# labgem/pangenomeNEM

Hardware: AMD Instinct MI355X
Metric: em_family_x_organism_cells_per_sec (higher is better)
Workload: dtype f32 chains with f64 intermediates (reference arithmetic); int32 popcounts in the M-step; 1 GPU; BASELINE configs[1]: 20000 families x 500 organisms, K=3, beta=0.5, contiguity graph (path + 5% chords, weights 1..8), ncem/sk_/pk; U-shaped family-frequency spectrum (Beta(0.3, 0.3) per family), default .m init; families_total=20000, families_per_gpu=20000, organisms=500, K=3, parallelism=1 GPU

## Files before the change

### include/nem_mi355x.h

```cpp
#ifndef NEM_MI355X_H
#define NEM_MI355X_H

#include <stdint.h>

#ifdef __cplusplus
extern "C" {
#endif

int nem(const char* Fname,
        const int nk,
        const char* algo,
        const float beta,
        const char* convergence,
        const float convergence_th,
        const char* format,
        const int it_max,
        const int dolog,
        const char* model_family,
        const char* proportion,
        const char* dispersion,
        const int init_mode);

typedef struct nemgpu_engine nemgpu_engine;

// ... 276 lines not shown
int nemgpu_ff_table(double l1, double l0, uint32_t* q0_256, uint32_t* q1_256);

float nemgpu_chain_host(const double* x, long long n, float init, int mode);
float nemgpu_repeat_add_host(float x, long long times, int mode);
int nemgpu_chain_device(const double* x, long long n, float init, int device, float* out);
float nemgpu_halfsum_host(const float* x, int n, int mode, int* stepped);
int nemgpu_halfsum_device(const float* x, int n, int waves, int device, float* out);
int nemgpu_halfsum_profile(const float* x, int n, int waves, int device, double us[5]);
int nemgpu_map_margin_host(const double* cinum, int n, int K, int* out);
int nemgpu_map_margin_device(const double* pkf, const float* ctx, int n, int K, float beta, int use_nei, int device, int* out);

void nemgpu_release_cached(void);

int nemgpu_set_graph_policy(nemgpu_engine* e, int capture_on_first);
int nemgpu_graph_counters(const nemgpu_engine* e, int out[4]);
int nemgpu_random_start_counters(const nemgpu_engine* e, int out[4]);

int nemgpu_set_stream(nemgpu_engine* e, void* hip_stream);

typedef struct nemgpu_gff nemgpu_gff;
int nemgpu_gff_info(int* tile_bytes, int* n_thresholds, int* thresholds);
int nemgpu_gff_create(nemgpu_gff** out, int device, const char* families_text, long long bytes, int hash_bits, int* n_families);
int nemgpu_gff_family_spans(const nemgpu_gff* h, int32_t* spans);
int nemgpu_gff_batch(nemgpu_gff* h, const char* text, long long bytes, const int32_t* file_start, const int32_t* file_end, int n_files,
                     int infer_singletons, int* n_genes, int* n_contigs, unsigned long long* error);
int nemgpu_gff_fetch(const nemgpu_gff* h, int32_t* file, int32_t* start, int32_t* end, int32_t* span_off, int32_t* span_len, int32_t* fam,
                     int32_t* contig, int32_t* fasta_off);
int nemgpu_gff_number(nemgpu_gff* h, const int32_t* name, const int32_t* org, int g, int n_names, int n_orgs, int lim_occurence, int32_t* genes,
                      int32_t* order, uint8_t* repeated, int* n_used);
int nemgpu_gff_stage_ms(const nemgpu_gff* h, float* ms);
// ... 7 lines not shown
```

### pangenomenem_amd/csrc/nem_engine.hip

```cpp
#include <hip/hip_runtime.h>
#include <dlfcn.h>
#include <pthread.h>
#include <unistd.h>

#include <algorithm>
#include <climits>
#include <atomic>
#include <cfloat>
#include <chrono>
#include <cmath>
#include <cstdio>
#include <cstdlib>
#include <cstring>
#include <condition_variable>
#include <deque>
#include <functional>
#include <map>
#include <string>
#include <mutex>
#include <thread>
#include <vector>

#include "nem_internal.hpp"
#include "nem_ff.hpp"
// ... 127 lines not shown
    double *crit2_lfi = nullptr, *crit2_lzi = nullptr;
    char* crit_pair_dev = nullptr;

    uint32_t sweep_counter = 0;
    int iters = 0, converged = 0, emptyk = 0, status = NEMGPU_OK;
    int zero_density = 0, first_zero = -1, sweep_rounds = 0;
    bool masks_valid = false;
    bool flags_clean = false;

    GraphCache batch_graphs{2 * 3 * 8 * 8, true, true};
    bool use_graphs = true;
    bool shadow_verify = true;
    int flag_sets = 1, fset = 0;
    bool round_counts = true;
    bool start_fused = true;
    int* stats_slot[2] = {};
    int* stats_last = nullptr;
    float* par_copy[3] = {}; double* pkfki_copy[3] = {}; float* logpkfki_copy[3] = {};
    int round_batch = 3;
    int rounds_iter = 2;
    int deep_iters = 2;
    uint8_t fz_need[kFzPositions] = {}; uint8_t fz_init_need = 0;
    int run_deep_used = 0; bool run_tracked = false;
    bool capture_first = false;
    int n_plain = 0, n_captured = 0, n_replayed = 0, n_host_rounds = 0;
    int ff_mode = -1;
    bool fused_update() const
    {
        return d <= kFusedMaxD && (cfg.disper == NEMGPU_DISP_KD || cfg.disper == NEMGPU_DISP_K_);
    }
// ... 441 lines not shown
    e->flags_clean = true;
    e->density_fresh = true;
    return NEMGPU_OK;
}

struct SweepCtx {
    SweepArgs a{};
    bool use_nei = false;
    bool multi = false;
    int r = 0;
    int checked = 0;
    int slot_base = 0;
    bool post = false; bool post_moved = false; CtrlArgs post_ctrl{};
    SweepArgs* hold = nullptr;
    int* count_into = nullptr;
};

int clear_sweep_flags(nemgpu_engine* e)
{
    if (current_recorder()) launch_fill(e->iter_flags() + FLAG_MOVED, kSweepFlagWords, 0, e->stream);
    else HIPCHK(hipMemsetAsync(e->iter_flags() + FLAG_MOVED, 0, kSweepFlagWords * sizeof(int), e->stream));
    e->flags_clean = true;
    return NEMGPU_OK;
}

int ensure_draw_window(nemgpu_engine* e, long lo, long count)
{
    if (e->draw_valid && e->draw_tab0 <= lo && lo + count <= e->draw_tab0 + e->draw_cap) return NEMGPU_OK;
    if (e->draw_borrowed) {
        e->draw_borrowed = false; e->draw_valid = false; e->draw_tab = nullptr; e->draw_cap = 0;
// ... 62 lines not shown
    const int r0 = c.r;
    for (int b = 0; b < count; b++, c.r++) {
        const int r = c.r;
        const int gb = (r == 0) ? P : ((r - 1) % 2 == 0 ? Q : R);
        const int ob = (r % 2 == 0) ? Q : R;
        if (ncem) {
            c.a.lab_old = e->lab[P]; c.a.lab_guess = e->lab[gb]; c.a.lab_out = e->lab[ob];
            c.a.tie_cnt_guess = e->tie_cnt[gb]; c.a.tie_cnt_out = e->tie_cnt[ob];
        } else { c.a.c_old = e->cbuf[P]; c.a.c_guess = e->cbuf[gb]; c.a.c_out = e->cbuf[ob]; }
        c.a.flags = e->round_flags(c.slot_base + r);
        c.a.fold_ticket = e->sweep_next + 32;
        c.a.prev_changed = (r == r0) ? nullptr : (e->round_flags(c.slot_base + r - 1) + FLAG_CHANGED);
        c.a.stop = e->stop_ptr;
        c.a.post_on = 0;
        c.a.post_stats = nullptr;
        if (c.hold != nullptr && c.post && ncem && r0 == 0 && count >= 2 && b >= count - 2) {
            c.a.post_on = 1; c.a.post_skip_guess = (r % 2 == 1) ? 1 : 0;
            c.a.post_nw64 = e->nw64; c.a.post_mask = e->mask; c.a.post_flags = e->iter_flags();
            if (b == count - 2) {
                c.a.post_from_guess = 0; c.a.post_moved = c.post_moved ? 1 : 0; c.a.post_no_masks = 0; c.a.post_ctrl = CtrlArgs{};
                if (c.count_into != nullptr) { c.a.post_stats = c.count_into; c.a.post_xt = e->xt; c.a.post_D = e->d; }
            } else {
                c.a.post_from_guess = 1; c.a.post_moved = 0; c.a.post_no_masks = 1; c.a.post_ctrl = c.post_ctrl;
                *c.hold = c.a;
                continue;
            }
        } else if (c.post && ncem && r0 == 0 && b == count - 1) {
            c.a.post_on = 1; c.a.post_from_guess = (r % 2 == 1) ? 1 : 0; c.a.post_moved = c.post_moved ? 1 : 0;
            c.a.post_skip_guess = c.a.post_from_guess;
            c.a.post_nw64 = e->nw64; c.a.post_mask = e->mask; c.a.post_flags = e->iter_flags(); c.a.post_ctrl = c.post_ctrl;
// ... 16 lines not shown
    a.pkfki = e->pkfki;
    a.tie_rule = e->cfg.tie_rule; a.tie_seed = e->cfg.tie_seed; a.map_full = e->map_margin ? 0 : 1; a.sweep_id = e->sweep_counter++;
    a.sweep_id_ptr = (e->stop_ptr != nullptr && !id_by_value) ? e->sweep_next : nullptr;
    if (e->libc()) {
        if (e->stop_ptr == nullptr) { int r = ensure_draw_window(e, e->draws, draw_need(e)); if (r) return r; }
        sweep_draw_args(e, a, e->stop_ptr == nullptr);
    }
    return NEMGPU_OK;
}

int sweep_enqueue(nemgpu_engine* e, float beta, SweepCtx& c, bool id_by_value = false, const CtrlArgs* post_ctrl = nullptr,
                  bool post_moved = false, int slot_base = 0, int rounds = 0, SweepArgs* hold = nullptr, int* count_into = nullptr)
{
    c = SweepCtx();
    c.slot_base = slot_base;
    if (post_ctrl != nullptr && e->ncem()) {
        c.post = true; c.post_moved = post_moved; c.post_ctrl = *post_ctrl; c.hold = hold;
        c.count_into = hold != nullptr ? count_into : nullptr;
    }
    { int r = sweep_setup(e, beta, c, id_by_value); if (r) return r; }
    if (!e->flags_clean) { int r = clear_sweep_flags(e); if (r) return r; }
    e->flags_clean = false;
    return sweep_launch_rounds(e, c, c.multi ? (rounds > 0 ? rounds : e->round_batch) : 1);
}

int sweep_complete(nemgpu_engine* e, SweepCtx& c, int* rounds_out, bool* extra, bool flags_ready = false, bool grow = false)
{
    int done_at = -1;
    if (extra) *extra = false;
    for (;;) {
// ... 205 lines not shown
{
    const char* v = getenv("NEM_MI355X_LIBC_INIT");
    return !(v && strcmp(v, "host") == 0);
}

static int init_beta_rounds(const nemgpu_engine* e)
{
    int n = std::max<int>(e->round_batch, (!e->ncem() && current_recorder() == nullptr) ? e->fz_init_need : 0);
    if (e->libc()) n = e->libc_rb;
    else if (e->ncem() && current_recorder() == nullptr && e->init_rounds_ncem >= 2) n = e->init_rounds_ncem;
    return n;
}

bool shadow_engine(const nemgpu_engine* e);

int enqueue_init(nemgpu_engine* e, bool defer_ctrl, SweepArgs* hold = nullptr, int* count_into = nullptr)
{
    int r;
    FinishArgs t = finish_args(e, 0, nullptr);
    t.reset_prop = e->prop0; t.reset_center = e->center0; t.reset_disp = e->disp0;
    t.reset_ctrl = e->ctrl(); t.reset_ctrl_words = C_WORDS; t.reset_sweep_next = e->sweep_next;
    if (hold != nullptr && count_into != nullptr) { t.zero_stats = count_into; t.n_zero_stats = e->k + e->k * e->d; }
    e->cur = 0;
    if (e->start_fused && shadow_engine(e)) {
        launch_density_start(t, e->xws, e->n, e->npad, e->pkfki, e->logpkfki, e->iter_flags() + FLAG_MOVED, kSweepFlagWords, e->stream);
        HIPCHK(hipGetLastError());
        e->tables_fresh = false;
        e->flags_clean = true; e->density_fresh = true;
    } else {
        launch_finish(t, e->stream);
        HIPCHK(hipGetLastError());
        e->tables_fresh = true; e->density_fresh = false;
        if ((r = do_density(e))) return r;
    }
    SweepCtx c0, c1;
    e->sweep_counter = 0;
    const bool libc = e->libc();
    const int ra = libc ? e->libc_ra : 1;
    if ((r = sweep_enqueue(e, 0.0f, c0, true, nullptr, false, kRoundCap - ra, libc ? ra : 0))) return r;
    e->flags_clean = true;
    e->cur = 1;
    CtrlArgs ca{};
    ca.ctrl = e->ctrl(); ca.iter_flags = e->iter_flags(); ca.round0 = e->round_flags(0); ca.n_rounds = init_beta_rounds(e);
    ca.param_fix = e->cfg.param_fix; ca.use_nei = ((e->has_graph && e->cfg.beta != 0.0f) || e->libc()) ? 1 : 0; ca.cvtest = e->cfg.cvtest;
    ca.ncem = e->ncem() ? 1 : 0; ca.cvthres = e->cfg.cvthres; ca.sweep_next = e->sweep_next; ca.ticket = e->sweep_next + 32;
    ca.draw_ctl = e->libc() ? e->draw_ctl : nullptr;
    ca.is_init = 1;
    ca.blind = e->round_flags(kRoundCap - ra);
    ca.blind_rounds = libc ? ra : 0;
    const bool defer = defer_ctrl && e->ncem() && !e->cfg.param_fix && hold == nullptr;
    CtrlArgs none{};
    if (libc) e->draw_extra_once = e->round_flags(kRoundCap - 1) + FLAG_NTIES;
    if ((r = sweep_enqueue(e, e->cfg.beta, c1, true, e->ncem() ? (defer ? &none : &ca) : nullptr, false, 0, ca.n_rounds, hold,
                           count_into))) return r;
// ... 488 lines not shown
    return enqueue();
}

int iterate_pipelined(nemgpu_engine* e, int n_iters, bool with_init)
{
    int r;
    LoopCursor lc;
    if ((r = loop_begin(e, lc, n_iters, with_init))) return r;
    if (lc.first && e->libc() && !libc_init_pipelined()) {
        if ((r = libc_init(e))) return r;
        lc.first = false;
    }
    while (loop_wants_batch(e, lc)) {
        if ((r = batch_plan(e, lc))) return r;
        const int cur0 = e->cur; const uint32_t sweep_counter0 = e->sweep_counter;
        Graphed how;
        r = run_graphed(e, lc.g < 8 ? &e->batch_graphs : nullptr, {(uint64_t)lc.batch_first, (uint64_t)lc.base, (uint64_t)lc.g, (uint64_t)lc.deep},
                        2, e->stream, [&]() { return batch_enqueue(e, lc, true); },
                        [&]() { e->cur = cur0; e->sweep_counter = sweep_counter0; }, &how);
        e->n_plain += how == Graphed::plain;
        e->n_captured += how == Graphed::captured;
        e->n_replayed += how == Graphed::replayed || (how == Graphed::captured && r == NEMGPU_OK);
        if (r) return r;
        HIPCHK(hipStreamSynchronize(e->stream));
        if ((r = batch_finish(e, lc))) return r;
    }
    return NEMGPU_OK;
}

int criteria(nemgpu_engine* e, float crit6[6], int buf);

int iterate_crit(nemgpu_engine* e, int n_iters, bool with_init)
{
    int r;
// ... 721 lines not shown
    e->n_total = n_total; e->n_true = n_total; e->d = d; e->k = k; e->lo = site_lo; e->hi = site_hi; e->n = site_hi - site_lo;
    e->device = device;
    e->npad = (e->n + 255) / 256 * 256;
    e->dpad = (d + 63) / 64 * 64;
    e->W = e->dpad / 32;
    e->wf = (d + 31) / 32;
    e->nw64 = (e->n + 63) / 64;
    e->cfg.algo = NEMGPU_ALGO_NCEM; e->cfg.beta = 0.5f; e->cfg.disper = NEMGPU_DISP_K_; e->cfg.propor = NEMGPU_PROP_K;
    e->cfg.cvtest = NEMGPU_CV_CLAS; e->cfg.cvthres = 1e-8f; e->cfg.it_max = 100; e->cfg.param_fix = 0;
    e->cfg.tie_rule = NEMGPU_TIE_HASH; e->cfg.tie_seed = 0;
    if (const char* g = getenv("NEM_MI355X_GRAPHS")) e->use_graphs = (g[0] != '0');
    if (const char* g = getenv("NEM_MI355X_SHADOW_VERIFY")) e->shadow_verify = (g[0] != '0');
    e->flag_sets = e->shadow_verify ? 3 : 1;
    if (const char* g = getenv("NEM_MI355X_ROUND_COUNTS")) e->round_counts = (g[0] != '0');
    if (const char* g = getenv("NEM_MI355X_START_FUSED")) e->start_fused = (g[0] != '0');
    if (const char* g = getenv("NEM_MI355X_ROUNDS")) e->round_batch = std::max(2, std::min(kRoundBatchMax, atoi(g)));
    if (const char* g = getenv("NEM_MI355X_ROUNDS_ITER")) e->rounds_iter = std::max(2, std::min(e->round_batch, atoi(g)));
    e->rounds_iter = std::min(e->rounds_iter, e->round_batch);
    if (const char* g = getenv("NEM_MI355X_FAULT_INJECT")) e->fault_inject = !strcmp(g, "fuzzy_pc") ? 1 : 0;
    if (const char* g = getenv("NEM_MI355X_FF")) e->ff_mode = (g[0] == '0') ? 0 : (g[0] == '1') ? 1 : -1;
    if (const char* g = getenv("NEM_MI355X_FF_BATCH")) e->ff_batch = (g[0] != '0');
    if (const char* g = getenv("NEM_MI355X_MAP_MARGIN")) e->map_margin = (g[0] != '0');
    if (const char* g = getenv("NEM_MI355X_SORT")) e->use_sort = (g[0] != '0');
    if (hip_stream) { e->stream = (hipStream_t)hip_stream; e->own_stream = false; }
    else {
        if (pool_stream_get(device, &e->stream) != hipSuccess) { delete e; set_error("hipStreamCreate failed"); return NEMGPU_E_DEVICE; }
        e->own_stream = true;
    }
    int r = NEMGPU_OK;
    alloc_for(e);
// ... 2791 lines not shown

int nemgpu_set_graph_policy(nemgpu_engine* e, int capture_on_first)
{
    if (!e) return NEMGPU_E_FUNCARG;
    e->capture_first = capture_on_first != 0;
    return NEMGPU_OK;
}

int nemgpu_graph_counters(const nemgpu_engine* e, int out[4])
{
    if (!e || !out) return NEMGPU_E_FUNCARG;
    out[0] = e->n_plain; out[1] = e->n_captured; out[2] = e->n_replayed; out[3] = e->n_host_rounds;
    return NEMGPU_OK;
}

int nemgpu_random_start_counters(const nemgpu_engine* e, int out[4])
{
    if (!e || !out) return NEMGPU_E_FUNCARG;
    out[0] = e->rs_rounds; out[1] = e->rs_lockstep; out[2] = e->rs_alone; out[3] = e->rs_redone;
    return NEMGPU_OK;
}

int nemgpu_set_stream(nemgpu_engine* e, void* hip_stream)
{
    if (!e || !hip_stream) return NEMGPU_E_FUNCARG;
    if (e->own_stream && e->stream) { (void)hipStreamSynchronize(e->stream); (void)hipStreamDestroy(e->stream); }
    e->stream = (hipStream_t)hip_stream;
    e->own_stream = false;
    drop_graphs(e);
    return NEMGPU_OK;
// ... 113 lines not shown
```

### pangenomenem_amd/csrc/nem_kernels.hpp

```cpp
#pragma once
#include <hip/hip_runtime.h>
#include <cstdint>
#include <cstring>
#include <type_traits>
#include <vector>

#include "../../include/nem_mi355x.h"

namespace nemk {

constexpr int kMaxKernelK = 32;
constexpr int kTicketWords = 32 * 33;
constexpr double kEpsilonD = 1e-20;

enum { FLAG_CHANGED = 0, FLAG_NZERO = 1, FLAG_FIRSTZERO = 2, FLAG_NTIES = 3, FLAG_ROUND_STRIDE = 4 };
enum { FLAG_EMPTYK = 0, FLAG_EMPTY_PROP = 1, FLAG_FAULT = 2, FLAG_MOVED = 3, FLAG_ITER_STRIDE = 4 };

enum { C_STOP = 0, C_FOLD = 1, C_ITERS = 10, C_COMMITS = 2, C_STATUS = 3, C_EMPTYK = 4, C_CONVERGED = 5, C_NEED_ROUNDS = 6,
       C_SWEEP_ROUNDS = 7, C_NZERO = 8, C_FIRSTZERO = 9, C_DRAWS = 11, C_DEEP = 12, C_DRAWS_INIT = 13, C_INIT_ROUNDS = 14, C_WORDS = 16 };

struct CtrlArgs {
    int* ctrl; const int* iter_flags; const int* round0;
    int n_rounds;
    int param_fix, use_nei, cvtest, ncem; float cvthres;
// ... 5 lines not shown
    const int* blind;
    int blind_rounds;
    int* draw_ctl;
    const uint8_t* q_tot;
};
void launch_ctrl(const CtrlArgs& a, hipStream_t s);

struct SweepArgs {
    int n_local, lo, n_total, K, npad, use_nei;
    const int* nei_ptr; const int* nei_idx; const float* nei_w;
    float beta;
    const double* pkfki;
    const uint8_t* lab_old; const uint8_t* lab_guess; uint8_t* lab_out;
    const float* c_old; const float* c_guess; float* c_out;
    int tie_rule; uint32_t tie_seed; uint32_t sweep_id;
    const int* sweep_id_ptr;
    int* flags;
    const int* prev_changed;
    const int* stop;
    const uint8_t* flags_in; int n_ranks, slot_stride, slot_pad;
    int post_on, post_from_guess, post_moved, post_nw64, post_skip_guess;
    int post_no_masks;
    uint64_t* post_mask; int* post_flags;
    CtrlArgs post_ctrl;
    uint8_t* publish_byte; int* publish_ticket;
    int* fold_ticket;
    const uint32_t* draw_tab; int draw_tab_len, draw_base, draw_tab0;
    const int* draw_ctl; const int* draw_extra;
    const int* tie_cnt_guess; int* tie_cnt_out;
    const uint8_t* rank_tot_in; int rank_index; uint8_t* rank_tot_out;
    int spb;
    int* post_stats; const uint64_t* post_xt; int post_D;
    int map_full;
};
struct LabelsPostArgs { int n_local, lo, K, nw64; const uint8_t* lab_new; const uint8_t* lab_old; uint64_t* mask; int* flags;
                        const int* stop; CtrlArgs ca; };
struct CountsArgs { int K, D, nw64; const uint64_t* xt; const uint64_t* mask; int* stats; const int* stop; CtrlArgs prev_ctrl; };
struct FuzzyArgs { int n, npad, K, D; const uint32_t* xw; const uint64_t* xt; int nw64; const float* c; float* nbobs_k;
                   float* in0; float* in1; float* inh_k; int* lastz; int* any1; float* center; float* iner; const int* stop;
                   float* ct; int ctpad;
                   float* chk;
                   int* fault;
                   int inject; };
struct ConvFuzzyArgs { size_t m; const float* c; const float* cold; float thres; int* flags; const int* stop; CtrlArgs ca; };
struct OnehotArgs { int n, K; const uint8_t* lab; float* c; };
struct CritArgs { int n, K, npad; const int* nei_ptr; const int* nei_idx; const float* nei_w; int use_nei; float beta;
// ... 121 lines not shown
```

### pangenomenem_amd/csrc/nem_sweep.hip

```cpp
#include <hip/hip_runtime.h>
#include <algorithm>
#include <cstdio>
#include <cstdlib>

#include "nem_kernels.hpp"
#include "nem_sweep_dev.hpp"

namespace nemk {

template <int KT, bool NCEM, int BS, bool LIBC = false, bool COUNT = false>
__global__ __launch_bounds__(BS) void k_sweep(SweepArgs a) { sweep_body<KT, NCEM, BS, LIBC, COUNT>(a, blockIdx.x, gridDim.x); }
template <int KT, bool NCEM, int BS, bool LIBC = false>
__global__ __launch_bounds__(BS) void k_sweep_b(const void* arr, int stride, const int* gx) { NEM_B_HEAD(SweepArgs) sweep_body<KT, NCEM, BS, LIBC>(a, blockIdx.x, nblk); }

static int sweep_variant(int K, bool ncem, bool big, bool libc) { return (K >= 1 && K <= 10 ? K : 0) | (ncem ? 16 : 0) | (big ? 32 : 0) | (libc && ncem ? 64 : 0); }

template <bool BATCHED>
static void sweep_dispatch(int variant, dim3 grid, unsigned bdim, hipStream_t s, const SweepArgs* a, const void* arr, int stride, const int* gx)
{
    const int kt = variant & 15; const bool ncem = (variant & 16) != 0, big = (variant & 32) != 0, libc = (variant & 64) != 0;
    dim3 block(bdim);
    auto launch = [&](auto KT, auto NC, auto BS, auto LC) {
        if (BATCHED) hipLaunchKernelGGL((k_sweep_b<decltype(KT)::value, decltype(NC)::value, decltype(BS)::value, decltype(LC)::value>), grid, block, 0, s, arr, stride, gx);
        else hipLaunchKernelGGL((k_sweep<decltype(KT)::value, decltype(NC)::value, decltype(BS)::value, decltype(LC)::value>), grid, block, 0, s, *a);
    };
    auto modes = [&](auto KT, auto BS) {
// ... 15 lines not shown
        const int per_block = (n_local + 256 * waves_of_blocks - 1) / (256 * waves_of_blocks);
        bs = std::min(1024, std::max(256, (per_block + 63) / 64 * 64));
    }
    if (big_out) *big_out = big;
    return bs;
}

void launch_sweep(const SweepArgs& a0, bool ncem, hipStream_t s)
{
    bool big = false;
    SweepArgs a = a0;
    const int bs = sweep_block_sites(a.n_local, a.K, &big);
    a.spb = big ? bs : 0;
    dim3 grid((a.n_local + bs - 1) / bs);
    const int variant = sweep_variant(a.K, ncem, big, a.tie_rule == NEMGPU_TIE_LIBC);
    if (a.post_stats != nullptr) {
        if (!(current_recorder() == nullptr && ncem && !big && a.K >= 1 && a.K <= 10 && a.tie_rule != NEMGPU_TIE_LIBC &&
              a.post_on && !a.post_no_masks && a.post_D >= 1 && a.post_D <= kFusedMaxD)) {
            fprintf(stderr, "launch_sweep: no counting round for this shape\n");
            abort();
        }
        dispatch_k<1, 10>(a.K, [&](auto KT) {
            hipLaunchKernelGGL((k_sweep<decltype(KT)::value, true, 256, false, true>), grid, dim3(256), 0, s, a);
        });
        return;
    }
    if (record_op(OP_SWEEP, variant, grid, (unsigned)bs, a)) return;
    sweep_dispatch<false>(variant, grid, (unsigned)bs, s, &a, nullptr, 0, nullptr);
}

// ... 49 lines not shown
```

### pangenomenem_amd/csrc/nem_sweep_dev.hpp

```cpp
#pragma once
#include <hip/hip_runtime.h>
#include <cstdint>

#include "nem_kernels.hpp"
#include "nem_map.hpp"

namespace nemk {

#ifdef NEM_PHASE_PROF
static __device__ unsigned long long g_sweep_phase[16];
#define NEM_SWEEP_PHASE(i) do { if (bx == 0 && threadIdx.x == 0) g_sweep_phase[(COUNT ? 8 : 0) + (i)] = wall_clock64(); } while (0)
#define NEM_SWEEP_PHASE_TAKE(t) const unsigned long long t = wall_clock64()
#define NEM_SWEEP_PHASE_PUT(i, t) do { if (bx == 0 && threadIdx.x == 0) g_sweep_phase[(COUNT ? 8 : 0) + (i)] = t; } while (0)
#else
#define NEM_SWEEP_PHASE(i) do { } while (0)
#define NEM_SWEEP_PHASE_TAKE(t) do { } while (0)
#define NEM_SWEEP_PHASE_PUT(i, t) do { } while (0)
#endif

__host__ __device__ inline uint32_t mix32(uint32_t seed, uint32_t sweep, uint32_t site)
{
    uint32_t h = seed * 0x9E3779B1u + sweep * 0x85EBCA77u + site * 0xC2B2AE3Du + 0x27D4EB2Fu;
    h ^= h >> 16; h *= 0x7FEB352Du;
    h ^= h >> 15; h *= 0x846CA68Bu;
// ... 243 lines not shown
constexpr int kLabMask = 0x7F, kLabDrew = 0x80;
constexpr int kTabShort = 1 << 30;
constexpr int kInnerCap = 64;

__device__ __forceinline__ int wave_sum_i32(int v)
{
    v += __builtin_amdgcn_update_dpp(0, v, 0xB1, 0xF, 0xF, false);
    v += __builtin_amdgcn_update_dpp(0, v, 0x4E, 0xF, 0xF, false);
    v += __builtin_amdgcn_update_dpp(0, v, 0x141, 0xF, 0xF, false);
    v += __builtin_amdgcn_update_dpp(0, v, 0x140, 0xF, 0xF, false);
    v += __builtin_amdgcn_update_dpp(0, v, 0x142, 0xA, 0xF, false);
    v += __builtin_amdgcn_update_dpp(0, v, 0x143, 0xC, 0xF, false);
    return __builtin_amdgcn_readlane(v, 63);
}

template <int KT, bool NCEM, int BS, bool LIBC = false, bool COUNT = false>
__device__ __forceinline__ void sweep_body(const SweepArgs& a, const int bx, const int nblk)
{
    static_assert(!COUNT || (NCEM && BS == 256 && !LIBC && KT > 0), "the counting round: NCEM, 256 sites per block");
    static_assert(C_STOP == 0 && C_FOLD == 1, "one 8-byte load");
    NEM_SWEEP_PHASE_TAKE(t_entry);
    const int spb = (BS > 256 && a.spb > 0) ? a.spb : BS;
    const int i = bx * spb + threadIdx.x;
    const bool active = (int)threadIdx.x < spb && i < a.n_local;
    const int gi = a.lo + (active ? i : 0);
    const int K = KT > 0 ? KT : a.K;
    constexpr int KA = KT > 0 ? KT : kMaxKernelK;
    int my_guess = 0, my_old = 0, my_new = 255;
    int blk_cnt_guess = 0;
    constexpr int kCntRows = COUNT ? kFusedMaxD / BS : 1;
    uint64_t xs[kCntRows][4];
    double pkf[NCEM ? KA : 1];
    int nb = 0, ne = 0;
    int fold_hint = 0;
// ... 4 lines not shown
            const int w0 = 4 * bx;
#pragma unroll
            for (int q = 0; q < kCntRows; q++) {
                const int d = (int)threadIdx.x + q * BS;
#pragma unroll
                for (int w = 0; w < 4; w++)
                    xs[q][w] = (d < a.post_D && w0 + w < a.post_nw64) ? a.post_xt[(size_t)d * a.post_nw64 + w0 + w] : 0ull;
            }
        }
#pragma unroll
        for (int k = 0; k < KA; k++) if (k < K) pkf[k] = active ? a.pkfki[(size_t)k * a.npad + i] : 0.0;
        if (active && a.use_nei) { nb = a.nei_ptr[i]; ne = a.nei_ptr[i + 1]; }
        const int* some = reinterpret_cast<const int*>(a.pkfki);
        int2 sf = *reinterpret_cast<const int2*>(a.stop != nullptr ? a.stop : some);
        int pc = *(a.prev_changed != nullptr ? a.prev_changed : some);
        if (active) { my_guess = a.lab_guess[gi]; my_old = a.lab_old[gi] & kLabMask; }
        if (a.stop == nullptr) sf = make_int2(0, 0);
        if (a.prev_changed == nullptr) pc = 1;
        __atomic_signal_fence(__ATOMIC_SEQ_CST);
        asm volatile("" :: "s"(pc));
        if (sf.x) return;
        fold_hint = sf.y;
        skip = (pc == 0);
    } else {
        if (a.stop != nullptr) {
            const int2 sf = *reinterpret_cast<const int2*>(a.stop);
            if (sf.x) return;
            fold_hint = sf.y;
        }
        skip = (a.prev_changed != nullptr && *a.prev_changed == 0);
    }
// ... 7 lines not shown
    if (skip && !(NCEM && a.post_on)) {
        if (a.publish_byte != nullptr && bx == 0 && threadIdx.x == 0) *a.publish_byte = 0;
        if (LIBC && a.prev_changed != nullptr && bx == 0 && threadIdx.x == 0) a.flags[FLAG_NTIES] = a.prev_changed[FLAG_NTIES - FLAG_CHANGED];
        return;
    }
    __shared__ int s_nzero, s_first;
    __shared__ int s_chg, s_mov;
    constexpr int kExpTab = 64;
    __shared__ double s_exp[NCEM ? kExpTab : 1];
    __shared__ __attribute__((aligned(16))) uint8_t s_lab[NCEM ? BS : 1];
    __shared__ uint64_t s_drew[BS / 64];
    bool zero_density = false;
    bool changed = false;
    __shared__ int s_anydrew;
    if (threadIdx.x == 0) { s_nzero = 0; s_first = 0; s_chg = 0; s_mov = 0; s_anydrew = 0; }
    if (NCEM) s_lab[threadIdx.x] = (uint8_t)my_guess;
    if (NCEM && a.use_nei && !skip && threadIdx.x < kExpTab) s_exp[threadIdx.x] = exp((double)a.beta * (double)(float)threadIdx.x);
    __shared__ int s_lower;
    if (LIBC && !skip && threadIdx.x < 64 && a.tie_cnt_guess != nullptr) {
        int part = 0;
        for (int b = threadIdx.x; b < bx; b += 64) part += a.tie_cnt_guess[b];
        part = wave_sum_i32(part);
        if (threadIdx.x == 0) {
            if (a.rank_tot_in != nullptr)
                for (int r = 0; r < a.rank_index; r++) part += *reinterpret_cast<const int*>(a.rank_tot_in + (size_t)r * a.slot_stride);
            s_lower = part;
        }
    }
    bool blk_drew = false;
    if (LIBC) blk_drew = __syncthreads_or((my_guess & kLabDrew) != 0) != 0;
// ... 3 lines not shown
    if (NCEM) {
    constexpr bool libc = LIBC;
    constexpr bool kMapShort = KT >= 1 && KT <= 7;
    const int blk_lo = a.lo + bx * spb;
    int dyn[4]; float wn[4]; int fl[4];
#pragma unroll
    for (int u = 0; u < 4; u++) { dyn[u] = -1; wn[u] = 0.0f; fl[u] = 255; }
    if (active && !skip && a.use_nei) {
        int jn[4];
#pragma unroll
        for (int u = 0; u < 4; u++) {
            const bool ok = nb + u < ne;
            jn[u] = ok ? a.nei_idx[nb + u] : gi;
            wn[u] = ok ? a.nei_w[nb + u] : 0.0f;
        }
#pragma unroll
        for (int u = 0; u < 4; u++) {
            if (nb + u < ne) {
                if (jn[u] < gi && jn[u] >= blk_lo) dyn[u] = jn[u] - blk_lo;
                else fl[u] = ((jn[u] < gi) ? a.lab_guess[jn[u]] : a.lab_old[jn[u]]) & kLabMask;
            }
        }
    }
    const bool long_row = ne - nb > 4;
    NEM_SWEEP_PHASE(3);
    int lower_draws = -1;
    bool tab_short = false;
    int cur = my_guess;
    int seen[4] = {-1, -1, -1, -1};
    uint64_t seen_drew = ~0ull; int seen_wave_draws = -1;
    for (int it = 0; it < kInnerCap; it++) {
        int below_in_block = 0;
        uint64_t drew_lt = 0;
        if (libc && blk_drew) {
            const uint64_t bal = __ballot((s_lab[threadIdx.x] & kLabDrew) != 0);
            if ((threadIdx.x & 63) == 0) s_drew[threadIdx.x >> 6] = bal;
// ... 17 lines not shown
                for (int k = 0; k < KA; k++) ctx[k] = 0.0f;
#pragma unroll
                for (int u = 0; u < 4; u++) {
                    seen[u] = lab[u];
                    if (nb + u < ne) {
#pragma unroll
                        for (int k = 0; k < KA; k++)
                            if (k < K) ctx[k] = ctx[k] + ((lab[u] == k) ? wn[u] : -0.0f);
                    }
                }
                for (int t = nb + 4; t < ne; t++) {
                    const int j = a.nei_idx[t];
                    const float wt = a.nei_w[t];
                    int l;
                    if (j < gi && j >= blk_lo) l = s_lab[j - blk_lo] & kLabMask;
                    else l = ((j < gi) ? a.lab_guess[j] : a.lab_old[j]) & kLabMask;
#pragma unroll
                    for (int k = 0; k < KA; k++)
                        if (k < K) ctx[k] = ctx[k] + ((l == k) ? wt : -0.0f);
                }
                float cf[KA];
                int kmax = 0;
                bool clear = false;
                if constexpr (kMapShort) {
                    double cinum[KA];
                    const double cum = local_cinum<KA>(a, K, pkf, ctx, cinum, s_exp, kExpTab);
                    zero_density = !(cum > 0);
                    clear = !a.map_full && map_clear_row<KA>(cinum, K, cum, kmax);
                    if (!clear) map_normalise<KA>(cinum, K, cum, cf);
                } else zero_density = local_proba<KA>(a, K, pkf, ctx, cf, s_exp, kExpTab);
// ... 99 lines not shown
    int post_lab = 255;
    if (NCEM && a.post_on) {
        int moved = 0;
        if (active) {
            if (skip) post_lab = (a.post_skip_guess ? my_guess : (int)a.lab_out[gi]) & kLabMask;
            else post_lab = a.post_from_guess ? (my_guess & kLabMask) : (my_new != 255 ? my_new : ((int)a.lab_out[gi] & kLabMask));
            if (a.post_moved) moved = (post_lab != my_old);
        }
        if (__any(moved) && (threadIdx.x & 63) == 0) s_mov = 1;
    }
    const uint64_t zmask = __ballot(zero_density);
    if (zmask != 0ull && (threadIdx.x & 63) == 0) {
        atomicAdd(&s_nzero, (int)__popcll(zmask));
        atomicMax(&s_first, a.n_total - (gi + (int)__ffsll((long long)zmask) - 1));
    }
    __syncthreads();
    NEM_SWEEP_PHASE(5);
    const bool fold = fold_hint != 0 && a.fold_ticket != nullptr && nblk > 32;
    if (threadIdx.x == 0 && s_nzero > 0) {
        if (!fold) atomicAdd(&a.flags[FLAG_NZERO], s_nzero);
        if (a.flags[FLAG_FIRSTZERO] < s_first) atomicMax(&a.flags[FLAG_FIRSTZERO], s_first);
    }
    constexpr int kNoLookBlocks = 128;
    if (threadIdx.x == 0) {
        const bool look = nblk > kNoLookBlocks;
        if (s_chg && !(look && __hip_atomic_load(&a.flags[FLAG_CHANGED], __ATOMIC_RELAXED, __HIP_MEMORY_SCOPE_AGENT) != 0))
            atomicOr(&a.flags[FLAG_CHANGED], 1);
        if (NCEM && a.post_on && s_mov && !(look && __hip_atomic_load(&a.post_flags[FLAG_MOVED], __ATOMIC_RELAXED, __HIP_MEMORY_SCOPE_AGENT) != 0))
            atomicOr(&a.post_flags[FLAG_MOVED], 1);
    }
    NEM_SWEEP_PHASE(6);
    __shared__ uint64_t s_cmask[COUNT ? KA : 1][4];
// ... 59 lines not shown
```

### pangenomenem_amd/engine.py

```python
import ctypes as C
import os

import numpy as np

_HERE = os.path.dirname(os.path.abspath(__file__))
LIB_PATH = os.environ.get("NEM_MI355X_LIB") or os.path.join(_HERE, "lib", "libnem_mi355x.so")

ALGO = {"nem": 0, "ncem": 1}
DISP = {"s__": 0, "sk_": 1, "s_d": 2, "skd": 3}
PROP = {"p_": 0, "pk": 1}
CVT = {"none": 0, "clas": 1, "crit": 2, "crit_logged": 3}
TIE = {"libc": 0, "first": 1, "hash": 2}
STATUS_OK, STATUS_W_EMPTYCLASS, STATUS_E_DEVICE, STATUS_E_INTERNAL = 0, 2, 9, 10


class NemGpuError(RuntimeError):
    pass


class Config(C.Structure):
    _fields_ = [("algo", C.c_int), ("beta", C.c_float), ("disper", C.c_int), ("propor", C.c_int),
                ("cvtest", C.c_int), ("cvthres", C.c_float), ("it_max", C.c_int), ("param_fix", C.c_int),
                ("tie_rule", C.c_int), ("tie_seed", C.c_uint32)]

# ... 67 lines not shown
    lib.nemgpu_get_labels.argtypes = [vp, vp]
    lib.nemgpu_get_params.argtypes = [vp, vp, vp, vp, vp]
    lib.nemgpu_get_results.argtypes = [vp, vp, vp, vp, vp, vp]
    lib.nemgpu_solve_many.argtypes = [vp, C.c_int, vp, C.c_int, C.c_int, C.c_int]
    lib.nemgpu_solve_many_devices.argtypes = [vp, C.c_int, vp, ip, C.c_int, C.c_int, C.c_int]
    lib.nemgpu_deal_groups.argtypes = [C.c_int, C.c_int, C.c_int, ip]
    lib.nemgpu_get_density.argtypes = [vp, vp, vp]
    lib.nemgpu_profile_density.argtypes = [vp, C.c_int, C.POINTER(C.c_double), C.POINTER(C.c_double), ip]
    lib.nemgpu_calibrate_fetch.argtypes = [C.c_size_t, C.c_int]
    lib.nemgpu_profile_kernels.argtypes = [vp, C.c_int, C.POINTER(C.c_double), C.POINTER(C.c_double), ip]
    lib.nemgpu_rccl_time_allgather.argtypes = [vp, vp, C.c_int, C.POINTER(C.c_double)]
    lib.nemgpu_set_stream.argtypes = [vp, vp]
    lib.nemgpu_set_fast_forward.argtypes = [vp, C.c_int]
    lib.nemgpu_set_graph_policy.argtypes = [vp, C.c_int]
    lib.nemgpu_graph_counters.argtypes = [vp, ip]
    lib.nemgpu_profile_density_many.argtypes = [C.POINTER(vp), C.c_int, C.c_int, C.POINTER(C.c_double), C.POINTER(C.c_double)]
    lib.nemgpu_random_start_counters.argtypes = [vp, ip]
    lib.nemgpu_rccl_ranks.argtypes = [vp]
    lib.nemgpu_rccl_selftest.argtypes = [vp, vp, C.c_int, C.c_int]
    lib.nemgpu_ff_table.argtypes = [C.c_double, C.c_double, vp, vp]
    lib.nemgpu_shard_end_enqueue.argtypes = [vp]
    lib.nemgpu_stats_words.argtypes = [vp]
    lib.nemgpu_shard_layout.argtypes = [vp, C.c_int, C.c_int, C.c_int, C.c_int, C.c_int]
    lib.nemgpu_shard_begin.argtypes = [vp]
    lib.nemgpu_shard_begin_restart.argtypes = [vp]
    lib.nemgpu_shard_estep_round1_counts.argtypes = [vp, C.c_float, C.c_int, vp, vp, vp, vp]
    lib.nemgpu_shard_mstep_partial.argtypes = [vp, vp, vp]
    lib.nemgpu_shard_counts.argtypes = [vp, vp]
    lib.nemgpu_rccl_open.argtypes = [C.c_char_p]
    lib.nemgpu_rccl_unique_id.argtypes = [vp]
# ... 353 lines not shown
        ms = C.c_double(0)
        self._chk(self.lib.nemgpu_rccl_time_allgather(self._h, C.c_void_p(buf_ptr), int(reps), C.byref(ms)))
        return ms.value

    def set_fast_forward(self, mode):
        self._chk(self.lib.nemgpu_set_fast_forward(self._h, int(mode)))

    def set_graph_policy(self, capture_on_first=True):
        self._chk(self.lib.nemgpu_set_graph_policy(self._h, int(bool(capture_on_first))))

    def graph_counters(self):
        out = (C.c_int * 4)()
        self._chk(self.lib.nemgpu_graph_counters(self._h, out))
        return dict(plain=out[0], captured=out[1], replayed=out[2], host_finished_sweeps=out[3])

    def random_start_counters(self):
        out = (C.c_int * 4)()
        self._chk(self.lib.nemgpu_random_start_counters(self._h, out))
        return dict(rounds=out[0], in_lockstep=out[1], alone=out[2], redone=out[3])

    def rccl_ranks(self):
        return int(self.lib.nemgpu_rccl_ranks(self._h))

    def set_stream(self, stream_ptr):
        self._chk(self.lib.nemgpu_set_stream(self._h, C.c_void_p(stream_ptr)))


def run_many(engines, fetch=True):
    if not engines:
        return []
# ... 83 lines not shown
```

Measured before the change: 386.9 billion cells/s.

## Fold the initial MAP labelling sweep into the first neighbourhood sweep

When enabled, initialisation no longer launches a separate sweep that turns the starting densities into labels. A new blind variant of the first sweep kernel computes each site's MAP label from the densities on the fly, including labels of out-of-block neighbours, and records the zero-density flags into the skipped sweep's flag slot. This removes one kernel launch and one label read/write pass per start, at the cost of redundant per-neighbour label recomputation. It is limited to K 2..7, at most 128 blocks and shadow engines, and aborts on unsupported shapes.

```diff
diff --git a/include/nem_mi355x.h b/include/nem_mi355x.h
--- a/include/nem_mi355x.h
+++ b/include/nem_mi355x.h
@@ -314,6 +314,7 @@
 
 int nemgpu_set_graph_policy(nemgpu_engine* e, int capture_on_first);
 int nemgpu_graph_counters(const nemgpu_engine* e, int out[4]);
+int nemgpu_debug_blind_folds(const nemgpu_engine* e);
 int nemgpu_random_start_counters(const nemgpu_engine* e, int out[4]);
 
 int nemgpu_set_stream(nemgpu_engine* e, void* hip_stream);
diff --git a/pangenomenem_amd/csrc/nem_engine.hip b/pangenomenem_amd/csrc/nem_engine.hip
--- a/pangenomenem_amd/csrc/nem_engine.hip
+++ b/pangenomenem_amd/csrc/nem_engine.hip
@@ -165,6 +165,10 @@
     int flag_sets = 1, fset = 0;
     bool round_counts = true;
     bool start_fused = true;
+    bool blind_fold = true;
+    int n_blind_folds = 0;
+    int blind_slot_once = -1; uint32_t blind_id_once = 0;
+
     int* stats_slot[2] = {};
     int* stats_last = nullptr;
     float* par_copy[3] = {}; double* pkfki_copy[3] = {}; float* logpkfki_copy[3] = {};
@@ -636,6 +640,7 @@
     bool post = false; bool post_moved = false; CtrlArgs post_ctrl{};
     SweepArgs* hold = nullptr;
     int* count_into = nullptr;
+    int blind_slot = -1; uint32_t blind_id = 0;
 };
 
 int clear_sweep_flags(nemgpu_engine* e)
@@ -728,6 +733,9 @@
         c.a.stop = e->stop_ptr;
         c.a.post_on = 0;
         c.a.post_stats = nullptr;
+        const bool blind = ncem && c.blind_slot >= 0 && r == 0;
+        c.a.blind_off = blind ? (int)(e->round_flags(c.blind_slot) - c.a.flags) : 0;
+        c.a.blind_sweep_id = blind ? c.blind_id : 0u;
         if (c.hold != nullptr && c.post && ncem && r0 == 0 && count >= 2 && b >= count - 2) {
             c.a.post_on = 1; c.a.post_skip_guess = (r % 2 == 1) ? 1 : 0;
             c.a.post_nw64 = e->nw64; c.a.post_mask = e->mask; c.a.post_flags = e->iter_flags();
@@ -774,6 +782,7 @@
 {
     c = SweepCtx();
     c.slot_base = slot_base;
+    c.blind_slot = e->blind_slot_once; c.blind_id = e->blind_id_once; e->blind_slot_once = -1;
     if (post_ctrl != nullptr && e->ncem()) {
         c.post = true; c.post_moved = post_moved; c.post_ctrl = *post_ctrl; c.hold = hold;
         c.count_into = hold != nullptr ? count_into : nullptr;
@@ -1009,6 +1018,13 @@
 
 bool shadow_engine(const nemgpu_engine* e);
 
+constexpr int kBlindFoldMaxBlocks = 128;
+static bool blind_fold_on(const nemgpu_engine* e)
+{
+    return e->blind_fold && e->start_fused && shadow_engine(e) && e->k >= 2 && e->k <= 7 &&
+           (e->n + 255) / 256 <= kBlindFoldMaxBlocks;
+}
+
 int enqueue_init(nemgpu_engine* e, bool defer_ctrl, SweepArgs* hold = nullptr, int* count_into = nullptr)
 {
     int r;
@@ -1032,7 +1048,11 @@
     e->sweep_counter = 0;
     const bool libc = e->libc();
     const int ra = libc ? e->libc_ra : 1;
-    if ((r = sweep_enqueue(e, 0.0f, c0, true, nullptr, false, kRoundCap - ra, libc ? ra : 0))) return r;
+    const bool fold = blind_fold_on(e);
+    if (fold) {
+        e->blind_slot_once = kRoundCap - ra; e->blind_id_once = e->sweep_counter++;
+        e->n_blind_folds++;
+    } else if ((r = sweep_enqueue(e, 0.0f, c0, true, nullptr, false, kRoundCap - ra, libc ? ra : 0))) return r;
     e->flags_clean = true;
     e->cur = 1;
     CtrlArgs ca{};
@@ -1551,10 +1571,12 @@
     while (loop_wants_batch(e, lc)) {
         if ((r = batch_plan(e, lc))) return r;
         const int cur0 = e->cur; const uint32_t sweep_counter0 = e->sweep_counter;
+        const int folds0 = e->n_blind_folds;
         Graphed how;
         r = run_graphed(e, lc.g < 8 ? &e->batch_graphs : nullptr, {(uint64_t)lc.batch_first, (uint64_t)lc.base, (uint64_t)lc.g, (uint64_t)lc.deep},
                         2, e->stream, [&]() { return batch_enqueue(e, lc, true); },
-                        [&]() { e->cur = cur0; e->sweep_counter = sweep_counter0; }, &how);
+                        [&]() { e->cur = cur0; e->sweep_counter = sweep_counter0; e->n_blind_folds = folds0; }, &how);
+        if (how == Graphed::replayed && lc.batch_first && blind_fold_on(e)) e->n_blind_folds++;
         e->n_plain += how == Graphed::plain;
         e->n_captured += how == Graphed::captured;
         e->n_replayed += how == Graphed::replayed || (how == Graphed::captured && r == NEMGPU_OK);
@@ -2306,6 +2328,7 @@
     e->flag_sets = e->shadow_verify ? 3 : 1;
     if (const char* g = getenv("NEM_MI355X_ROUND_COUNTS")) e->round_counts = (g[0] != '0');
     if (const char* g = getenv("NEM_MI355X_START_FUSED")) e->start_fused = (g[0] != '0');
+    if (const char* g = getenv("NEM_MI355X_BLIND_FOLD")) e->blind_fold = (g[0] != '0');
     if (const char* g = getenv("NEM_MI355X_ROUNDS")) e->round_batch = std::max(2, std::min(kRoundBatchMax, atoi(g)));
     if (const char* g = getenv("NEM_MI355X_ROUNDS_ITER")) e->rounds_iter = std::max(2, std::min(e->round_batch, atoi(g)));
     e->rounds_iter = std::min(e->rounds_iter, e->round_batch);
@@ -5127,6 +5150,11 @@
     return NEMGPU_OK;
 }
 
+int nemgpu_debug_blind_folds(const nemgpu_engine* e)
+{
+    return e ? e->n_blind_folds : -1;
+}
+
 int nemgpu_random_start_counters(const nemgpu_engine* e, int out[4])
 {
     if (!e || !out) return NEMGPU_E_FUNCARG;
diff --git a/pangenomenem_amd/csrc/nem_kernels.hpp b/pangenomenem_amd/csrc/nem_kernels.hpp
--- a/pangenomenem_amd/csrc/nem_kernels.hpp
+++ b/pangenomenem_amd/csrc/nem_kernels.hpp
@@ -43,6 +43,7 @@
     const uint8_t* lab_old; const uint8_t* lab_guess; uint8_t* lab_out;
     const float* c_old; const float* c_guess; float* c_out;
     int tie_rule; uint32_t tie_seed; uint32_t sweep_id;
+    uint32_t blind_sweep_id;
     const int* sweep_id_ptr;
     int* flags;
     const int* prev_changed;
@@ -59,6 +60,7 @@
     const int* tie_cnt_guess; int* tie_cnt_out;
     const uint8_t* rank_tot_in; int rank_index; uint8_t* rank_tot_out;
     int spb;
+    int blind_off;
     int* post_stats; const uint64_t* post_xt; int post_D;
     int map_full;
 };
diff --git a/pangenomenem_amd/csrc/nem_sweep.hip b/pangenomenem_amd/csrc/nem_sweep.hip
--- a/pangenomenem_amd/csrc/nem_sweep.hip
+++ b/pangenomenem_amd/csrc/nem_sweep.hip
@@ -10,6 +10,8 @@
 
 template <int KT, bool NCEM, int BS, bool LIBC = false, bool COUNT = false>
 __global__ __launch_bounds__(BS) void k_sweep(SweepArgs a) { sweep_body<KT, NCEM, BS, LIBC, COUNT>(a, blockIdx.x, gridDim.x); }
+template <int KT, bool COUNT>
+__global__ __launch_bounds__(256) void k_sweep_blind(SweepArgs a) { sweep_body<KT, true, 256, false, COUNT, true>(a, blockIdx.x, gridDim.x); }
 template <int KT, bool NCEM, int BS, bool LIBC = false>
 __global__ __launch_bounds__(BS) void k_sweep_b(const void* arr, int stride, const int* gx) { NEM_B_HEAD(SweepArgs) sweep_body<KT, NCEM, BS, LIBC>(a, blockIdx.x, nblk); }
 
@@ -55,6 +57,21 @@
     a.spb = big ? bs : 0;
     dim3 grid((a.n_local + bs - 1) / bs);
     const int variant = sweep_variant(a.K, ncem, big, a.tie_rule == NEMGPU_TIE_LIBC);
+    if (a.blind_off != 0) {
+        const bool count = a.post_stats != nullptr;
+        if (!(current_recorder() == nullptr && ncem && !big && a.K >= 2 && a.K <= 7 && a.tie_rule != NEMGPU_TIE_LIBC && a.use_nei &&
+              a.lo == 0 && a.slot_stride == 0 && a.flags_in == nullptr && a.prev_changed == nullptr &&
+              a.lab_guess != nullptr && a.lab_guess == a.lab_old && a.lab_out != a.lab_guess &&
+              (!count || (a.post_on && !a.post_no_masks && a.post_D >= 1 && a.post_D <= kFusedMaxD)))) {
+            fprintf(stderr, "launch_sweep: no blind round for this shape\n");
+            abort();
+        }
+        dispatch_k<2, 7>(a.K, [&](auto KT) {
+            if (count) hipLaunchKernelGGL((k_sweep_blind<decltype(KT)::value, true>), grid, dim3(256), 0, s, a);
+            else hipLaunchKernelGGL((k_sweep_blind<decltype(KT)::value, false>), grid, dim3(256), 0, s, a);
+        });
+        return;
+    }
     if (a.post_stats != nullptr) {
         if (!(current_recorder() == nullptr && ncem && !big && a.K >= 1 && a.K <= 10 && a.tie_rule != NEMGPU_TIE_LIBC &&
               a.post_on && !a.post_no_masks && a.post_D >= 1 && a.post_D <= kFusedMaxD)) {
diff --git a/pangenomenem_amd/csrc/nem_sweep_dev.hpp b/pangenomenem_amd/csrc/nem_sweep_dev.hpp
--- a/pangenomenem_amd/csrc/nem_sweep_dev.hpp
+++ b/pangenomenem_amd/csrc/nem_sweep_dev.hpp
@@ -281,10 +281,48 @@
     return __builtin_amdgcn_readlane(v, 63);
 }
 
-template <int KT, bool NCEM, int BS, bool LIBC = false, bool COUNT = false>
+template <int KA>
+__device__ __forceinline__ int blind_label(const SweepArgs& a, int K, const double* pkf, uint32_t site, bool* zero)
+{
+    double cinum[KA];
+    double cum = 0.0;
+#pragma unroll
+    for (int k = 0; k < KA; k++) {
+        if (k < K) {
+            const double v = pkf[k];
+            cinum[k] = v;
+            cum = cum + v;
+        }
+    }
+    *zero = !(cum > 0);
+    int kmax = 0;
+    if (!a.map_full && map_clear_row<KA>(cinum, K, cum, kmax)) return kmax;
+    float cf[KA];
+    map_normalise<KA>(cinum, K, cum, cf);
+    kmax = 0; float ukmax = cf[0];
+#pragma unroll
+    for (int k = 1; k < KA; k++) if (k < K && cf[k] > ukmax) { ukmax = cf[k]; kmax = k; }
+    if (a.tie_rule != NEMGPU_TIE_FIRST) {
+        int nequal = 0;
+#pragma unroll
+        for (int k = 1; k < KA; k++) if (k < K && k > kmax && cf[k] == ukmax) nequal++;
+        if (nequal > 0) {
+            const int pick = (int)(mix32(a.tie_seed, a.blind_sweep_id, site) % (uint32_t)(nequal + 1));
+            int seen_eq = 0, chosen = kmax;
+#pragma unroll
+            for (int k = 1; k < KA; k++)
+                if (k < K && k > kmax && cf[k] == ukmax) { seen_eq++; if (seen_eq == pick) chosen = k; }
+            kmax = chosen;
+        }
+    }
+    return kmax;
+}
+
+template <int KT, bool NCEM, int BS, bool LIBC = false, bool COUNT = false, bool BLIND = false>
 __device__ __forceinline__ void sweep_body(const SweepArgs& a, const int bx, const int nblk)
 {
     static_assert(!COUNT || (NCEM && BS == 256 && !LIBC && KT > 0), "the counting round: NCEM, 256 sites per block");
+    static_assert(!BLIND || (NCEM && BS == 256 && !LIBC && KT >= 2 && KT <= 7), "the blind round: NCEM, 256 sites per block, K = 2 .. 7");
     static_assert(C_STOP == 0 && C_FOLD == 1, "one 8-byte load");
     NEM_SWEEP_PHASE_TAKE(t_entry);
     const int spb = (BS > 256 && a.spb > 0) ? a.spb : BS;
@@ -319,7 +357,7 @@
         const int* some = reinterpret_cast<const int*>(a.pkfki);
         int2 sf = *reinterpret_cast<const int2*>(a.stop != nullptr ? a.stop : some);
         int pc = *(a.prev_changed != nullptr ? a.prev_changed : some);
-        if (active) { my_guess = a.lab_guess[gi]; my_old = a.lab_old[gi] & kLabMask; }
+        if constexpr (!BLIND) { if (active) { my_guess = a.lab_guess[gi]; my_old = a.lab_old[gi] & kLabMask; } }
         if (a.stop == nullptr) sf = make_int2(0, 0);
         if (a.prev_changed == nullptr) pc = 1;
         __atomic_signal_fence(__ATOMIC_SEQ_CST);
@@ -357,6 +395,18 @@
     bool changed = false;
     __shared__ int s_anydrew;
     if (threadIdx.x == 0) { s_nzero = 0; s_first = 0; s_chg = 0; s_mov = 0; s_anydrew = 0; }
+    __shared__ __attribute__((aligned(16))) uint8_t s_old[BLIND ? BS : 1];
+    __shared__ int s_bnzero, s_bfirst;
+    bool blind_zero = false;
+    if constexpr (BLIND) {
+        if (threadIdx.x == 0) { s_bnzero = 0; s_bfirst = 0; }
+        bool z;
+        my_guess = blind_label<KA>(a, K, pkf, (uint32_t)gi, &z);
+        my_old = my_guess;
+        blind_zero = active && z;
+        s_old[threadIdx.x] = (uint8_t)my_guess;
+        if (active) const_cast<uint8_t*>(a.lab_guess)[gi] = (uint8_t)my_guess;
+    }
     if (NCEM) s_lab[threadIdx.x] = (uint8_t)my_guess;
     if (NCEM && a.use_nei && !skip && threadIdx.x < kExpTab) s_exp[threadIdx.x] = exp((double)a.beta * (double)(float)threadIdx.x);
     __shared__ int s_lower;
@@ -390,12 +440,31 @@
             jn[u] = ok ? a.nei_idx[nb + u] : gi;
             wn[u] = ok ? a.nei_w[nb + u] : 0.0f;
         }
+        if constexpr (BLIND) {
+            bool far[4];
+            double pn[4][KA];
+#pragma unroll
+            for (int u = 0; u < 4; u++) far[u] = nb + u < ne && (jn[u] < blk_lo || jn[u] >= blk_lo + BS);
+#pragma unroll
+            for (int u = 0; u < 4; u++)
+#pragma unroll
+                for (int k = 0; k < KA; k++) pn[u][k] = far[u] ? a.pkfki[(size_t)k * a.npad + (jn[u] - a.lo)] : 0.0;
+#pragma unroll
+            for (int u = 0; u < 4; u++) {
+                if (nb + u < ne) {
+                    if (jn[u] < gi && jn[u] >= blk_lo) dyn[u] = jn[u] - blk_lo;
+                    else if (!far[u]) fl[u] = s_old[jn[u] - blk_lo];
+                    else { bool z; fl[u] = blind_label<KA>(a, K, pn[u], (uint32_t)jn[u], &z); }
+                }
+            }
+        } else {
 #pragma unroll
         for (int u = 0; u < 4; u++) {
             if (nb + u < ne) {
                 if (jn[u] < gi && jn[u] >= blk_lo) dyn[u] = jn[u] - blk_lo;
                 else fl[u] = ((jn[u] < gi) ? a.lab_guess[jn[u]] : a.lab_old[jn[u]]) & kLabMask;
             }
+        }
         }
     }
     const bool long_row = ne - nb > 4;
@@ -443,6 +512,16 @@
                     const float wt = a.nei_w[t];
                     int l;
                     if (j < gi && j >= blk_lo) l = s_lab[j - blk_lo] & kLabMask;
+                    else if constexpr (BLIND) {
+                        if (j >= blk_lo && j < blk_lo + BS) l = s_old[j - blk_lo];
+                        else {
+                            double pj[KA];
+#pragma unroll
+                            for (int k = 0; k < KA; k++) pj[k] = a.pkfki[(size_t)k * a.npad + (j - a.lo)];
+                            bool z;
+                            l = blind_label<KA>(a, K, pj, (uint32_t)j, &z);
+                        }
+                    }
                     else l = ((j < gi) ? a.lab_guess[j] : a.lab_old[j]) & kLabMask;
 #pragma unroll
                     for (int k = 0; k < KA; k++)
@@ -572,8 +651,20 @@
         atomicAdd(&s_nzero, (int)__popcll(zmask));
         atomicMax(&s_first, a.n_total - (gi + (int)__ffsll((long long)zmask) - 1));
     }
+    if constexpr (BLIND) {
+        const uint64_t bmask = __ballot(blind_zero);
+        if (bmask != 0ull && (threadIdx.x & 63) == 0) {
+            atomicAdd(&s_bnzero, (int)__popcll(bmask));
+            atomicMax(&s_bfirst, a.n_total - (gi + (int)__ffsll((long long)bmask) - 1));
+        }
+    }
     __syncthreads();
     NEM_SWEEP_PHASE(5);
+    if (BLIND && threadIdx.x == 0 && s_bnzero > 0) {
+        int* bf = a.flags + a.blind_off;
+        atomicAdd(&bf[FLAG_NZERO], s_bnzero);
+        if (bf[FLAG_FIRSTZERO] < s_bfirst) atomicMax(&bf[FLAG_FIRSTZERO], s_bfirst);
+    }
     const bool fold = fold_hint != 0 && a.fold_ticket != nullptr && nblk > 32;
     if (threadIdx.x == 0 && s_nzero > 0) {
         if (!fold) atomicAdd(&a.flags[FLAG_NZERO], s_nzero);
diff --git a/pangenomenem_amd/engine.py b/pangenomenem_amd/engine.py
--- a/pangenomenem_amd/engine.py
+++ b/pangenomenem_amd/engine.py
@@ -105,6 +105,8 @@
     lib.nemgpu_set_fast_forward.argtypes = [vp, C.c_int]
     lib.nemgpu_set_graph_policy.argtypes = [vp, C.c_int]
     lib.nemgpu_graph_counters.argtypes = [vp, ip]
+    if hasattr(lib, "nemgpu_debug_blind_folds"):
+        lib.nemgpu_debug_blind_folds.argtypes = [vp]
     lib.nemgpu_profile_density_many.argtypes = [C.POINTER(vp), C.c_int, C.c_int, C.POINTER(C.c_double), C.POINTER(C.c_double)]
     lib.nemgpu_random_start_counters.argtypes = [vp, ip]
     lib.nemgpu_rccl_ranks.argtypes = [vp]
@@ -488,6 +490,9 @@
         self._chk(self.lib.nemgpu_graph_counters(self._h, out))
         return dict(plain=out[0], captured=out[1], replayed=out[2], host_finished_sweeps=out[3])
 
+    def blind_folds(self):
+        return int(self.lib.nemgpu_debug_blind_folds(self._h)) if hasattr(self.lib, "nemgpu_debug_blind_folds") else 0
+
     def random_start_counters(self):
         out = (C.c_int * 4)()
         self._chk(self.lib.nemgpu_random_start_counters(self._h, out))
```

After: 393.2 billion cells/s, median of 6. 1.6% higher.
